# hangxu0304/DeepReduce

Measured on NVIDIA H100. Metric: ResNet-50 images/sec (whole job, device-timed, max over ranks), higher is better.
Workload: dtype bf16

## Files before the change

deepreduce_b200/models/fused_bn.py:

```python
from __future__ import annotations

import os

import torch
import torch.nn as nn
import torch.nn.functional as F


def enabled() -> bool:
    return os.environ.get("DR_FUSED_BN", "1") != "0"


def _eligible_x(x: torch.Tensor) -> bool:
    return (x.is_cuda and x.dtype == torch.bfloat16 and x.dim() == 4 and x.stride(1) == 1
            and x.is_contiguous(memory_format=torch.channels_last) and x.size(1) % 8 == 0 and x.size(1) <= 8192
            and x.numel() < 2 ** 31 - 1 and x.numel() // x.size(1) > 1)


def _eligible_bn(bn: nn.BatchNorm2d) -> bool:
    return (bn.training and bn.track_running_stats and bn.running_mean is not None and bn.momentum is not None
            and bn.affine)


def eligible(x: torch.Tensor, bn: nn.BatchNorm2d) -> bool:
# ... 25 lines not shown
        dx, dw, db = ops.cuda_module().bn_backward(0, _grad(gy), mask, x, [mean, invstd, weight])
        return dx, dw, db, None, None


class _BNAddReLU(torch.autograd.Function):

    @staticmethod
    def forward(ctx, x, weight, bias, mean, invstd, z, wz, bz, mz, iz):
        from .. import ops
        mod = ops.cuda_module()
        if wz is None:
            o, mask = mod.bn_apply(1, x, [mean, invstd, weight, bias], z)
            ctx.save_for_backward(x, weight, mean, invstd, mask)
        else:
            o, mask = mod.bn_apply(2, x, [mean, invstd, weight, bias], z, [mz, iz, wz, bz])
            ctx.save_for_backward(x, weight, mean, invstd, mask, z, wz, mz, iz)
        ctx.has_bn_z = wz is not None
        return o

    @staticmethod
    def backward(ctx, go):
        from .. import ops
        mod = ops.cuda_module()
        saved = ctx.saved_tensors
        x, weight, mean, invstd, mask = saved[:5]
        if not ctx.has_bn_z:
            dx, dw, db, g = mod.bn_backward(1, _grad(go), mask, x, [mean, invstd, weight])
            return dx, dw, db, None, None, g, None, None, None, None
        z, wz, mz, iz = saved[5:]
        dx, dw, db, dz, dwz, dbz = mod.bn_backward(2, _grad(go), mask, x, [mean, invstd, weight], z, [mz, iz, wz])
        return dx, dw, db, None, None, dz, dwz, dbz, None, None


def bn_relu(x: torch.Tensor, bn: nn.BatchNorm2d) -> torch.Tensor:
    if not eligible(x, bn):
        return F.relu(bn(x), inplace=True)
    mean, invstd = _stats(x, bn)
    return _BNReLU.apply(x, bn.weight, bn.bias, mean, invstd)


def bn_add_relu(x: torch.Tensor, bn: nn.BatchNorm2d, idt: torch.Tensor) -> torch.Tensor:
    if not (eligible(x, bn) and idt.dtype == x.dtype and idt.shape == x.shape and idt.stride() == x.stride()):
        return F.relu(bn(x) + idt, inplace=True)
    mean, invstd = _stats(x, bn)
    return _BNAddReLU.apply(x, bn.weight, bn.bias, mean, invstd, idt, None, None, None, None)


def bn_bn_add_relu(x: torch.Tensor, bn: nn.BatchNorm2d, xd: torch.Tensor, bnd: nn.BatchNorm2d) -> torch.Tensor:
    if not (eligible(x, bn) and eligible(xd, bnd) and xd.shape == x.shape and xd.stride() == x.stride()):
        return F.relu(bn(x) + bnd(xd), inplace=True)
    md, id_ = _stats(xd, bnd)
    mean, invstd = _stats(x, bn)
    return _BNAddReLU.apply(x, bn.weight, bn.bias, mean, invstd, xd, bnd.weight, bnd.bias, md, id_)
```

deepreduce_b200/models/resnet.py:

```python
from __future__ import annotations

import torch.nn as nn
import torch.nn.functional as F

from .fused_bn import bn_add_relu, bn_bn_add_relu, bn_relu


class _BasicCifar(nn.Module):
    def __init__(self, inp, out, stride):
        super().__init__()
        self.conv1 = nn.Conv2d(inp, out, 3, stride, 1, bias=False)
        self.bn1 = nn.BatchNorm2d(out)
        self.conv2 = nn.Conv2d(out, out, 3, 1, 1, bias=False)
        self.bn2 = nn.BatchNorm2d(out)
        self.pad = None
        if stride != 1 or inp != out:
            self.pad = (out - inp, stride)

    def forward(self, x):
        y = F.relu(self.bn1(self.conv1(x)))
        y = self.bn2(self.conv2(y))
        if self.pad is not None:
            extra, s = self.pad
            x = F.pad(x[:, :, ::s, ::s], (0, 0, 0, 0, extra // 2, extra - extra // 2))
        return F.relu(x + y)


class ResNetCifar(nn.Module):
    def __init__(self, n: int = 3, num_classes: int = 10):
        super().__init__()
        self.conv1 = nn.Conv2d(3, 16, 3, 1, 1, bias=False)
        self.bn1 = nn.BatchNorm2d(16)
        layers, inp = [], 16
        for out, stride in ((16, 1), (32, 2), (64, 2)):
            for i in range(n):
                layers.append(_BasicCifar(inp, out, stride if i == 0 else 1))
                inp = out
        self.layers = nn.Sequential(*layers)
# ... 25 lines not shown
        self.downsample = None
        if downsample:
            self.downsample = nn.Sequential(nn.Conv2d(inp, out, 1, stride, bias=False), nn.BatchNorm2d(out))

    def forward(self, x):
        xd = None if self.downsample is None else self.downsample[0](x)
        y = bn_relu(self.conv1(x), self.bn1)
        y = bn_relu(self.conv2(y), self.bn2)
        y = self.conv3(y)
        if xd is None:
            return bn_add_relu(y, self.bn3, x)
        return bn_bn_add_relu(y, self.bn3, xd, self.downsample[1])


class ResNet(nn.Module):
    def __init__(self, blocks=(3, 4, 6, 3), num_classes: int = 1000):
        super().__init__()
        self.conv1 = nn.Conv2d(3, 64, 7, 2, 3, bias=False)
        self.bn1 = nn.BatchNorm2d(64)
        self.maxpool = nn.MaxPool2d(3, 2, 1)
        stages, inp = [], 64
        for i, (n, width) in enumerate(zip(blocks, (64, 128, 256, 512))):
            for j in range(n):
                stride = 2 if (j == 0 and i > 0) else 1
                stages.append(_Bottleneck(inp, width, stride, downsample=(j == 0)))
                inp = width * 4
        self.layers = nn.Sequential(*stages)
        self.fc = nn.Linear(inp, num_classes)
        for m in self.modules():
            if isinstance(m, nn.Conv2d):
                nn.init.kaiming_normal_(m.weight, mode="fan_out", nonlinearity="relu")

    def forward(self, x):
        x = self.maxpool(bn_relu(self.conv1(x), self.bn1))
        x = self.layers(x)
        x = F.adaptive_avg_pool2d(x, 1).flatten(1)
        return self.fc(x)


def resnet50(num_classes: int = 1000) -> ResNet:
    return ResNet((3, 4, 6, 3), num_classes)
```

deepreduce_b200/ops/csrc/binding.cpp:

```cpp
#include <ATen/cuda/CUDAContext.h>
#include <c10/cuda/CUDAGuard.h>
#include <c10/cuda/CUDAStream.h>
#include <torch/extension.h>

#include <condition_variable>
#include <deque>
#include <mutex>
#include <thread>

#include "ops.h"

namespace py = pybind11;
using dr::EngineParams;

#define CHECK_CUDA_T(x) TORCH_CHECK((x).is_cuda() && (x).is_contiguous(), #x " must be a contiguous CUDA tensor")

static cudaStream_t cur_stream() { return at::cuda::getCurrentCUDAStream().stream(); }

static void check_last(const char* what) {
  cudaError_t e = cudaGetLastError();
  TORCH_CHECK(e == cudaSuccess, what, ": ", cudaGetErrorString(e));
}

static torch::Tensor bloom_insert(torch::Tensor idx, int64_t k, int64_t m_bits, int64_t seed) {
// ... 260 lines not shown
  for (int i = 0; i < 4; ++i) check_chan(p[i], C, names[i]);
  return {p[0].data_ptr<float>(), p[1].data_ptr<float>(), p[2].data_ptr<float>(), p[3].data_ptr<float>()};
}

static void check_like_x(const torch::Tensor& t, const torch::Tensor& x, const char* what) {
  TORCH_CHECK(t.sizes() == x.sizes() && t.strides() == x.strides() && t.scalar_type() == torch::kBFloat16 &&
                  t.device() == x.device(),
              "bn: ", what, " must match x in shape, layout, dtype and device");
}

static std::vector<torch::Tensor> bn_apply(int64_t mode, torch::Tensor x, std::vector<torch::Tensor> p,
                                           c10::optional<torch::Tensor> z, std::vector<torch::Tensor> pz) {
  check_bn_input(x);
  const int64_t C = x.size(1);
  const dr::BnParams px = bn_params(p, C);
  dr::BnParams pzz{};
  const void* zp = nullptr;
  if (mode != 0) {
    TORCH_CHECK(z.has_value(), "bn: mode ", mode, " needs z");
    check_like_x(*z, x, "z");
    zp = z->data_ptr();
    if (mode == 2) pzz = bn_params(pz, C);
  }
  c10::cuda::CUDAGuard g(x.device());
  const int64_t rows = x.numel() / C;
  auto out = torch::empty_like(x);
  auto mask = torch::empty({rows, C / 8}, x.options().dtype(torch::kUInt8));
  cudaError_t e = dr::launch_bn_apply((int)mode, x.data_ptr(), px, zp, pzz, out.data_ptr(), mask.data_ptr(), rows,
                                      (int)C, cur_stream());
  TORCH_CHECK(e == cudaSuccess, "bn_apply: ", cudaGetErrorString(e));
  return {out, mask};
}

static dr::BnParams bn_bwd_params(const std::vector<torch::Tensor>& p, int64_t C) {
  TORCH_CHECK(p.size() == 3, "bn_backward: expected (mean, invstd, weight)");
  const char* names[3] = {"mean", "invstd", "weight"};
  for (int i = 0; i < 3; ++i) check_chan(p[i], C, names[i]);
  return {p[0].data_ptr<float>(), p[1].data_ptr<float>(), p[2].data_ptr<float>(), nullptr};
}

static std::vector<torch::Tensor> bn_backward(int64_t mode, torch::Tensor go, torch::Tensor mask, torch::Tensor x,
                                              std::vector<torch::Tensor> p, c10::optional<torch::Tensor> z,
                                              std::vector<torch::Tensor> pz) {
  TORCH_CHECK(mode >= 0 && mode <= 2, "bn_backward: mode must be 0, 1 or 2");
  check_bn_input(x);
  TORCH_CHECK(go.sizes() == x.sizes() && go.scalar_type() == torch::kBFloat16 && go.device() == x.device() &&
                  go.is_contiguous(at::MemoryFormat::ChannelsLast),
              "bn_backward: go must be a channels_last bf16 tensor of x's shape on x's device");
  const int64_t C = x.size(1), rows = x.numel() / C;
  TORCH_CHECK(mask.is_cuda() && mask.scalar_type() == torch::kUInt8 && mask.is_contiguous() &&
                  mask.numel() == rows * (C / 8) && mask.device() == x.device(),
              "bn_backward: mask must be bn_apply's mask for x");
  c10::cuda::CUDAGuard guard(x.device());
  int block_y = 0, grid_y = 0;
  dr::bn_row_tree(rows, (int)C, &block_y, &grid_y);
  TORCH_CHECK((int64_t)block_y * grid_y <= rows, "bn_backward: reduction tree wider than the rows");
  const int n_sums = mode == 2 ? 3 : 2;
  auto f32 = x.options().dtype(torch::kFloat32);
  auto sums = torch::empty({n_sums, C}, f32);
  auto staging = grid_y > 1 ? torch::empty({n_sums, grid_y, C}, f32) : torch::Tensor();
  auto dx = torch::empty_like(x), dw = torch::empty({C}, f32), db = torch::empty({C}, f32);
  dr::BnBwd b{};
  b.go = go.data_ptr(); b.mask = mask.data_ptr<uint8_t>(); b.x = x.data_ptr();
  b.px = bn_bwd_params(p, C);
  b.dx = dx.data_ptr(); b.sums = sums.data_ptr<float>(); b.staging = grid_y > 1 ? staging.data_ptr<float>() : nullptr;
  b.dw = dw.data_ptr<float>(); b.db = db.data_ptr<float>();
  std::vector<torch::Tensor> res{dx, dw, db};
  if (mode == 1) {
    auto g = torch::empty_like(x);
    b.g = g.data_ptr();
    res.push_back(g);
  } else if (mode == 2) {
    TORCH_CHECK(z.has_value(), "bn_backward: mode 2 needs z");
    check_like_x(*z, x, "z");
    b.z = z->data_ptr();
    b.pz = bn_bwd_params(pz, C);
    auto dz = torch::empty_like(x), dwz = torch::empty({C}, f32), dbz = torch::empty({C}, f32);
    b.dz = dz.data_ptr(); b.dwz = dwz.data_ptr<float>(); b.dbz = dbz.data_ptr<float>();
    res.insert(res.end(), {dz, dwz, dbz});
  }
  cudaError_t e = dr::launch_bn_backward((int)mode, b, rows, (int)C, cur_stream());
  TORCH_CHECK(e == cudaSuccess, "bn_backward: ", cudaGetErrorString(e));
  return res;
}

struct Engine {
  EngineParams P{};
  int grid = 0;
  int grid_cap = 0;
  int blocks_per_sm = 2;
  int dyn_smem = 64 * 1024;
  int device = 0;

  Engine(int64_t tensors, int64_t tiles, int64_t n_tensors, int64_t n_tiles, int64_t slot_words,
         int64_t payload_words, int64_t grad, int64_t resid, int64_t hist, int64_t hist_total, int64_t sel,
         int64_t tile_count, int64_t barrier, int64_t status, std::vector<int64_t> arenas, int rank, int world) {
    TORCH_CHECK(world <= dr::kMaxWorld && (int)arenas.size() == world, "bad world/arenas");
    P.tensors = reinterpret_cast<const dr::TensorDesc*>(tensors);
    P.tiles = reinterpret_cast<const dr::TileInfo*>(tiles);
    P.n_tensors = (uint32_t)n_tensors; P.n_tiles = (uint32_t)n_tiles;
    P.slot_words = (uint32_t)slot_words; P.payload_words = (uint32_t)payload_words;
    P.grad = reinterpret_cast<float*>(grad); P.resid = reinterpret_cast<float*>(resid);
    P.hist = reinterpret_cast<uint32_t*>(hist); P.hist_total = reinterpret_cast<uint32_t*>(hist_total);
    P.sel = reinterpret_cast<dr::SelState*>(sel);
// ... 168 lines not shown
}
static int64_t arena_import(const std::string& b) {
  TORCH_CHECK(b.size() == sizeof(dr::ArenaHandle), "bad handle");
  dr::ArenaHandle h;
  memcpy(h.bytes, b.data(), sizeof(h.bytes));
  void* p = dr::arena_import(h);
  TORCH_CHECK(p != nullptr, "cudaIpcOpenMemHandle failed (peer access / IPC unavailable)");
  return (int64_t)p;
}
static torch::Tensor arena_as_tensor(int64_t p, int64_t n_words, int64_t device) {
  auto opts = torch::TensorOptions().dtype(torch::kInt32).device(torch::kCUDA, (int)device);
  return torch::from_blob((void*)p, {n_words}, opts);
}

PYBIND11_MODULE(TORCH_EXTENSION_NAME, m) {
  m.def("launch_count", [] { return (int64_t)dr::launch_count(); });
  m.def("bloom_insert", &bloom_insert);
  m.def("bloom_select", &bloom_select);
  m.def("qsgd_encode", &qsgd_encode);
  m.def("qsgd_decode", &qsgd_decode);
  m.def("pack_bits", &pack_bits);
  m.def("unpack_bits", &unpack_bits);
  m.def("polyfit_fit", &polyfit_fit);
  m.def("polyfit_eval", &polyfit_eval);
  m.def("dexp_fit", &dexp_fit);
  m.def("conflict_sets_pick", &conflict_sets_pick);
  m.def("delta_bp128_encode", &delta_bp128_encode);
  m.def("delta_bp128_decode", &delta_bp128_decode);
  m.def("u8_to_nhwc_norm", &u8_to_nhwc_norm);
  m.def("bn_stats", &bn_stats, py::arg("x"), py::arg("running_mean"), py::arg("running_var"), py::arg("momentum"),
        py::arg("eps"), py::arg("torch_kernel") = false);
  m.def("bn_apply", &bn_apply, py::arg("mode"), py::arg("x"), py::arg("p"), py::arg("z") = py::none(),
        py::arg("pz") = std::vector<torch::Tensor>{});
  m.def("bn_backward", &bn_backward, py::arg("mode"), py::arg("go"), py::arg("mask"), py::arg("x"), py::arg("p"),
        py::arg("z") = py::none(), py::arg("pz") = std::vector<torch::Tensor>{});
  m.def("rle_runs", &rle_runs);
  m.def("rle_indices", &rle_indices);
  m.def("arena_alloc", &arena_alloc);
  m.def("arena_free", [](int64_t p) { dr::arena_free((void*)p); });
  m.def("arena_export", &arena_export);
  m.def("arena_import", &arena_import);
  m.def("arena_close", [](int64_t p) { dr::arena_close((void*)p); });
  m.def("arena_as_tensor", &arena_as_tensor);
  m.def("enable_peer_access", [](std::vector<int> devices) { return dr::arena_enable_peer_access(devices.data(), (int)devices.size()); });
  m.attr("TILE") = dr::kTile;
  m.attr("ARENA_HDR_WORDS") = dr::kArenaHdrWords;
  m.attr("SLOT_HEADER_WORDS") = dr::kSlotHeaderWords;
  m.attr("HIST_BINS") = dr::kHistBins;
  m.attr("NUM_HIST") = dr::kNumHist;
  m.attr("PH_END") = (int)dr::kPhEnd;

  py::class_<Engine>(m, "Engine")
      .def(py::init<int64_t, int64_t, int64_t, int64_t, int64_t, int64_t, int64_t, int64_t, int64_t, int64_t, int64_t,
                    int64_t, int64_t, int64_t, std::vector<int64_t>, int, int>())
      .def("configure", &Engine::configure)
      .def("set_buffers", &Engine::set_buffers)
      .def("set_poly", &Engine::set_poly)
      .def("set_shard", &Engine::set_shard)
      .def("set_has_rle", &Engine::set_has_rle)
      .def("set_scratch", &Engine::set_scratch)
      .def("set_peer_timeout_ms", &Engine::set_peer_timeout_ms)
      .def("set_fault", &Engine::set_fault)
      .def("set_deterministic", &Engine::set_deterministic)
      .def("set_cost_prefix", &Engine::set_cost_prefix)
      .def("set_debug_times", &Engine::set_debug_times)
      .def("set_cuts", &Engine::set_cuts)
// ... 12 lines not shown
```

deepreduce_b200/ops/csrc/bn.cu:

```cuda
#include <cuda_bf16.h>

#include <algorithm>

#include "common.cuh"
#include "ops.h"

namespace dr {

namespace {

constexpr int kVec = 8;
constexpr int kApplyThreads = 256;
constexpr int kReduceThreads = 128;

struct ChanParams {
  float m[kVec], inv[kVec], w[kVec], b[kVec];
};

__device__ __forceinline__ void load8(const float* __restrict__ p, float* d) {
  const float4 a = __ldg(reinterpret_cast<const float4*>(p));
  const float4 b = __ldg(reinterpret_cast<const float4*>(p) + 1);
  d[0] = a.x; d[1] = a.y; d[2] = a.z; d[3] = a.w;
  d[4] = b.x; d[5] = b.y; d[6] = b.z; d[7] = b.w;
}
// ... 25 lines not shown
  const int c = (threadIdx.x % groups) * kVec;
  ChanParams a;
  load_params(px, c, a);
  ChanParams d;
  if (kMode == 2) load_params(pz, c, d);
  const int64_t step = (int64_t)gridDim.x * rows_per_cta;
#pragma unroll 2
  for (int64_t r = (int64_t)blockIdx.x * rows_per_cta + rsub; r < rows; r += step) {
    const int64_t off = r * C + c;
    const uint4 vx = *reinterpret_cast<const uint4*>(x + off);
    uint4 vz = make_uint4(0, 0, 0, 0);
    if (kMode != 0) vz = *reinterpret_cast<const uint4*>(z + off);
    const __nv_bfloat16* hx = reinterpret_cast<const __nv_bfloat16*>(&vx);
    const __nv_bfloat16* hz = reinterpret_cast<const __nv_bfloat16*>(&vz);
    uint4 vo;
    __nv_bfloat16* ho = reinterpret_cast<__nv_bfloat16*>(&vo);
    unsigned bits = 0;
#pragma unroll
    for (int i = 0; i < kVec; ++i) {
      __nv_bfloat16 y = __float2bfloat16_rn(bn_elem(__bfloat162float(hx[i]), a.m[i], a.inv[i], a.w[i], a.b[i]));
      if (kMode != 0) {
        const __nv_bfloat16 s = kMode == 1 ? hz[i]
                                           : __float2bfloat16_rn(bn_elem(__bfloat162float(hz[i]), d.m[i], d.inv[i], d.w[i], d.b[i]));
        y = __float2bfloat16_rn(__fadd_rn(__bfloat162float(y), __bfloat162float(s)));
      }
      ho[i] = relu_bf16(y);
      bits |= (__bfloat162float(ho[i]) <= 0.f ? 0u : 1u) << i;
    }
    *reinterpret_cast<uint4*>(out + off) = vo;
    mask[r * groups + c / kVec] = (uint8_t)bits;
  }
}

struct RowTree {
  int block_y, grid_y;
  __host__ __device__ int S() const { return block_y * grid_y; }
  __host__ __device__ int loops(int rows) const { return 1 + (rows - 1) / (S() * kLoads); }
  static constexpr int kLoads = 4;
};

constexpr int kStatsThreads = 256;

__device__ __forceinline__ void welford_update(float x, float inv, float valid, float& mean, float& m2n) {
  const float d0 = __fsub_rn(x, mean);
  mean = __fmaf_rn(d0, inv, mean);
  const float d1 = __fsub_rn(x, mean);
  m2n = __fmaf_rn(__fmul_rn(d0, d1), valid, m2n);
}

template <int kN, bool kFuseNew>
__device__ __forceinline__ void welford_merge(int& n, float* mean, float* m2n, int n_new, const float* mean_new,
                                              const float* m2n_new) {
  const float fn = (float)n, fn_new = (float)n_new;
  const float factor = __frcp_rn((float)max(1, n + n_new));
#pragma unroll
  for (int i = 0; i < kN; ++i) {
    const float d = __fsub_rn(mean[i], mean_new[i]);
    const float s = kFuseNew ? __fmaf_rn(mean_new[i], fn_new, __fmul_rn(mean[i], fn))
                             : __fmaf_rn(mean[i], fn, __fmul_rn(mean_new[i], fn_new));
    mean[i] = __fmul_rn(s, factor);
    const float u = __fmul_rn(__fmul_rn(__fmul_rn(d, d), fn_new), fn);
    m2n[i] = __fadd_rn(m2n[i], __fmaf_rn(u, factor, m2n_new[i]));
  }
  n += n_new;
}

// ... 183 lines not shown
  const int group = blockIdx.x * gpc + tg;
  const bool live = group * kVec < C;
  const int c = live ? group * kVec : 0;
  const int S = t.S();
  float m[kVec], mz[kVec];
#pragma unroll
  for (int i = 0; i < kVec; ++i) {
    m[i] = mean[c + i];
    mz[i] = kMode == 2 ? mean_z[c + i] : 0.f;
  }
  float acc[kSums][L][kVec];
#pragma unroll
  for (int k = 0; k < kSums; ++k)
#pragma unroll
    for (int j = 0; j < L; ++j)
#pragma unroll
      for (int i = 0; i < kVec; ++i) acc[k][j][i] = 0.f;
  const int mgroups = C / kVec;
  int r = blockIdx.y * t.block_y + y;
  const int n_loops = t.loops(rows);
  struct Batch {
    uint4 g[L], x[L], z[L];
    unsigned m[L];
  };
  auto load = [&](Batch& b, int r0) {
#pragma unroll
    for (int j = 0; j < L; ++j) {
      const int rr = r0 + j * S;
      if (live && rr < rows) {
        const int off = rr * C + c;
        b.g[j] = *reinterpret_cast<const uint4*>(go + off);
        b.x[j] = *reinterpret_cast<const uint4*>(x + off);
        if (kMode == 2) b.z[j] = *reinterpret_cast<const uint4*>(z + off);
        b.m[j] = mask[rr * mgroups + group];
      } else {
        b.g[j] = uint4{}; b.x[j] = uint4{}; b.z[j] = uint4{}; b.m[j] = 0;
      }
    }
  };
  Batch cur;
  load(cur, r);
  for (int it = 0; it < n_loops; ++it) {
    Batch nxt;
    load(nxt, r + L * S);
    const unsigned* mb = cur.m;
#pragma unroll
    for (int j = 0; j < L; ++j) {
      const __nv_bfloat16* hg = reinterpret_cast<const __nv_bfloat16*>(&cur.g[j]);
      const __nv_bfloat16* hx = reinterpret_cast<const __nv_bfloat16*>(&cur.x[j]);
      const __nv_bfloat16* hz = reinterpret_cast<const __nv_bfloat16*>(&cur.z[j]);
      uint4 vo;
      __nv_bfloat16* ho = reinterpret_cast<__nv_bfloat16*>(&vo);
#pragma unroll
      for (int i = 0; i < kVec; ++i) {
        const unsigned bit = (mb[j] >> i) & 1u;
        const float g = masked(hg[i], bit);
        if (kMode == 1) ho[i] = bit ? hg[i] : __float2bfloat16_rn(0.f);
        acc[0][j][i] = __fadd_rn(acc[0][j][i], g);
        acc[1][j][i] = __fmaf_rn(__fsub_rn(__bfloat162float(hx[i]), m[i]), g, acc[1][j][i]);
        if (kMode == 2) acc[2][j][i] = __fmaf_rn(__fsub_rn(__bfloat162float(hz[i]), mz[i]), g, acc[2][j][i]);
      }
      if (kMode == 1 && live && r + j * S < rows) *reinterpret_cast<uint4*>(g_out + (r + j * S) * C + c) = vo;
    }
    cur = nxt;
    r += L * S;
  }
#pragma unroll
  for (int k = 0; k < kSums; ++k) {
#pragma unroll
    for (int i = 0; i < kVec; ++i)
#pragma unroll
      for (int j = 1; j < L; ++j) acc[k][0][i] = __fadd_rn(acc[k][0][i], acc[k][j][i]);
    tree_over_y<kVec>(acc[k][0], sh, y, t.block_y, tg * kVec, gpc * kVec);
  }
  if (y != 0 || !live) return;
#pragma unroll
  for (int k = 0; k < kSums; ++k)
#pragma unroll
    for (int i = 0; i < kVec; ++i) {
      if (t.grid_y > 1) o.staging[((size_t)k * t.grid_y + blockIdx.y) * C + c + i] = acc[k][0][i];
      else bwd_store(o, k, c + i, C, acc[k][0][i], invstd, invstd_z);
    }
}

__global__ void bn_bwd_finalize_kernel(BwdOut o, RowTree t, int n_sums, int C, const float* __restrict__ invstd,
                                       const float* __restrict__ invstd_z) {
  extern __shared__ float sh[];
  const int cols = blockDim.x / t.block_y;
  const int col = threadIdx.x % cols, y = threadIdx.x / cols;
// ... 28 lines not shown

__device__ __forceinline__ __nv_bfloat16 elemt(float g, float x, const ElemtChan& p, int i, float norm) {
  const float a = __fmaf_rn(-p.sdy[i], norm, g);
  return __float2bfloat16_rn(__fmul_rn(__fmaf_rn(-p.f1[i], __fsub_rn(x, p.m[i]), a), p.f2[i]));
}

struct ElemtArgs {
  const float *mean, *invstd, *weight, *sums;
  const float *mean_z, *invstd_z, *weight_z;
};

template <int kMode>
__global__ void __launch_bounds__(kApplyThreads) bn_bwd_elemt_kernel(const __nv_bfloat16* __restrict__ g_in,
                                                                     const uint8_t* __restrict__ mask,
                                                                     const __nv_bfloat16* __restrict__ x,
                                                                     const __nv_bfloat16* __restrict__ z, ElemtArgs a,
                                                                     __nv_bfloat16* __restrict__ dx,
                                                                     __nv_bfloat16* __restrict__ dz, float norm,
                                                                     int64_t rows, int C) {
  const int groups = C / kVec;
  const int rows_per_cta = blockDim.x / groups;
  const int rsub = threadIdx.x / groups;
  if (rsub >= rows_per_cta) return;
  const int c = (threadIdx.x % groups) * kVec;
  ElemtChan p;
  elemt_params(a.mean, a.invstd, a.weight, a.sums, a.sums + C, norm, c, p);
  ElemtChan q;
  if (kMode == 2) elemt_params(a.mean_z, a.invstd_z, a.weight_z, a.sums, a.sums + 2 * C, norm, c, q);
  const int64_t step = (int64_t)gridDim.x * rows_per_cta;
#pragma unroll 2
  for (int64_t r = (int64_t)blockIdx.x * rows_per_cta + rsub; r < rows; r += step) {
    const int64_t off = r * C + c;
    const uint4 vg = *reinterpret_cast<const uint4*>(g_in + off);
    const uint4 vx = *reinterpret_cast<const uint4*>(x + off);
    uint4 vz = make_uint4(0, 0, 0, 0);
    if (kMode == 2) vz = *reinterpret_cast<const uint4*>(z + off);
    const unsigned mb = kMode == 1 ? 0xffu : mask[r * groups + c / kVec];
    const __nv_bfloat16* hg = reinterpret_cast<const __nv_bfloat16*>(&vg);
    const __nv_bfloat16* hx = reinterpret_cast<const __nv_bfloat16*>(&vx);
    const __nv_bfloat16* hz = reinterpret_cast<const __nv_bfloat16*>(&vz);
    uint4 vo, vd;
    __nv_bfloat16* ho = reinterpret_cast<__nv_bfloat16*>(&vo);
    __nv_bfloat16* hd = reinterpret_cast<__nv_bfloat16*>(&vd);
#pragma unroll
    for (int i = 0; i < kVec; ++i) {
      const float g = masked(hg[i], (mb >> i) & 1u);
      ho[i] = elemt(g, __bfloat162float(hx[i]), p, i, norm);
      if (kMode == 2) hd[i] = elemt(g, __bfloat162float(hz[i]), q, i, norm);
    }
    *reinterpret_cast<uint4*>(dx + off) = vo;
    if (kMode == 2) *reinterpret_cast<uint4*>(dz + off) = vd;
  }
}

__global__ void bn_update_stats_kernel(const float* __restrict__ mean, float* __restrict__ var_invstd,
                                       float* __restrict__ running_mean, float* __restrict__ running_var, int C,
                                       float momentum, float bessel, float eps) {
  const int c = blockIdx.x * blockDim.x + threadIdx.x;
  if (c >= C) return;
  const float m = mean[c], v = var_invstd[c];
  const float unbiased_var = v * bessel;
  running_mean[c] = m * momentum + (1 - momentum) * running_mean[c];
  running_var[c] = unbiased_var * momentum + (1 - momentum) * running_var[c];
  var_invstd[c] = rsqrtf(v + eps);
}

template <typename K>
cudaError_t rows_grid(K kernel, int64_t rows, int C, int& grid, int& threads) {
  const int groups = C / kVec;
  const int rows_per_cta = groups >= kApplyThreads ? 1 : kApplyThreads / groups;
// ... 27 lines not shown
  return std::max<int>(1, (int)(n - (n >> 1)));
}

RowTree row_tree(int rows, int C) {
  const int block_x = std::min(last_pow2((unsigned)C), 32);
  const int block_y = std::min(last_pow2((unsigned)((rows + 15) / 16)), 512 / block_x);
  int grid_y = std::min((rows + block_y * 16 - 1) / (block_y * 16), 128);
  if (grid_y < 8) grid_y = 1;
  return {block_y, grid_y};
}

template <int kMode>
cudaError_t launch_bwd_reduce(const BnBwd& b, const RowTree& t, const BwdOut& o, int rows, int C, cudaStream_t st) {
  const int groups = C / kVec;
  const int gpc = std::min(groups, std::max(1, kReduceThreads / t.block_y));
  const dim3 grid((groups + gpc - 1) / gpc, t.grid_y);
  const int threads = gpc * t.block_y;
  count_launch();
  bn_bwd_reduce_kernel<kMode><<<grid, threads, threads * kVec * sizeof(float), st>>>(
      reinterpret_cast<const __nv_bfloat16*>(b.go), b.mask, reinterpret_cast<const __nv_bfloat16*>(b.x), b.px.mean,
      b.px.invstd, reinterpret_cast<const __nv_bfloat16*>(b.z), b.pz.mean, b.pz.invstd,
      reinterpret_cast<__nv_bfloat16*>(b.g), o, t, rows, C);
  return cudaGetLastError();
}

template <int kMode>
cudaError_t launch_bwd_elemt(const BnBwd& b, const ElemtArgs& a, int64_t rows, int C, cudaStream_t st) {
  int grid = 0, threads = 0;
  cudaError_t e = rows_grid(bn_bwd_elemt_kernel<kMode>, rows, C, grid, threads);
  if (e != cudaSuccess) return e;
  const float norm = (float)(1.0 / (double)rows);
  count_launch();
  bn_bwd_elemt_kernel<kMode><<<grid, threads, 0, st>>>(
      reinterpret_cast<const __nv_bfloat16*>(kMode == 1 ? b.g : b.go), b.mask,
      reinterpret_cast<const __nv_bfloat16*>(b.x), reinterpret_cast<const __nv_bfloat16*>(b.z), a,
      reinterpret_cast<__nv_bfloat16*>(b.dx), reinterpret_cast<__nv_bfloat16*>(b.dz), norm, rows, C);
  return cudaGetLastError();
}

template <int kMode>
cudaError_t launch_backward(const BnBwd& b, int64_t rows64, int C, cudaStream_t st) {
  const int rows = (int)rows64;
  const RowTree t = row_tree(rows, C);
  const BwdOut o{b.sums, b.dw, b.db, b.dwz, b.dbz, b.staging};
  cudaError_t e = launch_bwd_reduce<kMode>(b, t, o, rows, C, st);
  if (e != cudaSuccess) return e;
  if (t.grid_y > 1) {
    const int cols = std::max(1, 512 / t.block_y);
    const int threads = cols * t.block_y;
    count_launch();
    bn_bwd_finalize_kernel<<<(C + cols - 1) / cols, threads, threads * sizeof(float), st>>>(
        o, t, kMode == 2 ? 3 : 2, C, b.px.invstd, b.pz.invstd);
    e = cudaGetLastError();
    if (e != cudaSuccess) return e;
  }
  const ElemtArgs a{b.px.mean, b.px.invstd, b.px.weight, b.sums, b.pz.mean, b.pz.invstd, b.pz.weight};
  return launch_bwd_elemt<kMode>(b, a, rows64, C, st);
}

cudaError_t launch_stats(const BnStats& s, int rows, int C, cudaStream_t st) {
  const RowTree t = row_tree(rows, C);
  const int grid_y = t.grid_y;
  const StatsOut o{s.mean, s.invstd, s.running_mean, s.running_var,
                   s.staging, s.staging + (size_t)grid_y * C, reinterpret_cast<int*>(s.staging + 2 * (size_t)grid_y * C),
                   s.momentum, s.bessel, s.eps};
  const int groups = C / kVec;
  const int gpc = std::min(groups, std::max(1, kStatsThreads / (RowTree::kLoads * t.block_y)));
  const int threads = gpc * RowTree::kLoads * t.block_y;
  count_launch();
  bn_stats_kernel<<<dim3((groups + gpc - 1) / gpc, grid_y), threads, WelfordSlots<kVec>::bytes(threads), st>>>(
      reinterpret_cast<const __nv_bfloat16*>(s.x), o, t, rows, C);
  cudaError_t e = cudaGetLastError();
  if (e != cudaSuccess || grid_y == 1) return e;
  const int cols = std::max(1, 512 / t.block_y);
  const int fthreads = cols * t.block_y;
  count_launch();
  bn_stats_finalize_kernel<<<(C + cols - 1) / cols, fthreads, WelfordSlots<1>::bytes(fthreads), st>>>(o, t, C);
  return cudaGetLastError();
}

}

void bn_row_tree(int64_t rows, int C, int* block_y, int* grid_y) {
  const RowTree t = row_tree((int)rows, C);
  *block_y = t.block_y;
  *grid_y = t.grid_y;
}

cudaError_t launch_bn_backward(int mode, const BnBwd& b, int64_t rows, int C, cudaStream_t st) {
  if (rows == 0) return cudaSuccess;
  switch (mode) {
    case 0: return launch_backward<0>(b, rows, C, st);
    case 1: return launch_backward<1>(b, rows, C, st);
    case 2: return launch_backward<2>(b, rows, C, st);
    default: return cudaErrorInvalidValue;
  }
}

cudaError_t launch_bn_stats(const BnStats& s, int64_t rows, int C, cudaStream_t st) {
  if (rows == 0) return cudaSuccess;
  return launch_stats(s, (int)rows, C, st);
}

cudaError_t launch_bn_update_stats(const float* mean, float* var_invstd, float* running_mean, float* running_var, int C,
                                   float momentum, float bessel, float eps, cudaStream_t st) {
  count_launch();
  bn_update_stats_kernel<<<(C + 255) / 256, 256, 0, st>>>(mean, var_invstd, running_mean, running_var, C, momentum,
                                                          bessel, eps);
  return cudaGetLastError();
}

cudaError_t launch_bn_apply(int mode, const void* x, const BnParams& px, const void* z, const BnParams& pz, void* out,
                            void* mask, int64_t rows, int C, cudaStream_t st) {
  switch (mode) {
    case 0: return launch_apply<0>(x, px, z, pz, out, mask, rows, C, st);
    case 1: return launch_apply<1>(x, px, z, pz, out, mask, rows, C, st);
    case 2: return launch_apply<2>(x, px, z, pz, out, mask, rows, C, st);
    default: return cudaErrorInvalidValue;
  }
}

}
```

deepreduce_b200/ops/csrc/ops.h:

```cpp
#pragma once
#include <cuda_runtime.h>
#include <stdint.h>

#include "plan.h"

namespace dr {

int engine_max_grid(int blocks_per_sm, int dyn_smem_bytes);
cudaError_t engine_launch(const EngineParams& P, int grid, int blocks_per_sm, int dyn_smem_bytes, cudaStream_t stream);
void count_launch(int n);
long long launch_count();

void launch_bloom_insert(const int64_t* idx, int64_t n, uint32_t* filter, uint32_t n_hash, uint32_t m_bits,
                         uint32_t seed, cudaStream_t st);
void launch_bloom_count(const uint32_t* filter, uint32_t d, uint32_t n_hash, uint32_t m_bits, uint32_t seed,
                        uint32_t* tile_counts, uint32_t* tile_excl, cudaStream_t st);
void launch_bloom_emit(const uint32_t* filter, uint32_t d, uint32_t n_hash, uint32_t m_bits, uint32_t seed,
                       const uint32_t* tile_excl, int64_t* out, uint32_t limit, cudaStream_t st);
void launch_qsgd_encode(const float* v, int64_t K, int bucket, int q, uint32_t seed, void* lvl, bool i16, float* norms,
                        cudaStream_t st);
void launch_qsgd_decode(const void* lvl, bool i16, const float* norms, int64_t K, int bucket, int q, float* out,
                        cudaStream_t st);
void launch_pack_bits(const int64_t* vals, int64_t n, int bits, uint32_t* out, int64_t n_words, cudaStream_t st);
void launch_unpack_bits(const uint32_t* in, int64_t n_words, int64_t n, int bits, int64_t* out, cudaStream_t st);
// ... 7 lines not shown
void launch_bp128_widths(const int64_t* idx, int64_t n, uint32_t* widths, cudaStream_t st);
void launch_bp128_pack(const int64_t* idx, int64_t n, const uint32_t* widths, const int64_t* word_off, uint32_t* out,
                       cudaStream_t st);
void launch_bp128_unpack(const uint32_t* in, int64_t n, int64_t* word_off, int64_t* deltas, cudaStream_t st);
void launch_rle_count(const int64_t* idx, int64_t n, uint32_t* counts, uint32_t* excl, cudaStream_t st);
void launch_rle_runs(const int64_t* idx, int64_t n, const uint32_t* excl, int64_t* start_pos, int64_t* end_pos,
                     int64_t n_runs, int64_t d, int64_t* runs, cudaStream_t st);
void launch_rle_expand(const int64_t* ones_excl, const int64_t* run_start, int64_t n_runs, int64_t total, int64_t* out,
                       cudaStream_t st);

struct ArenaHandle { unsigned char bytes[64]; };
void* arena_alloc(size_t bytes);
void arena_free(void* p);
ArenaHandle arena_export(void* p);
void* arena_import(const ArenaHandle& h);
void arena_close(void* p);
int arena_enable_peer_access(const int* devices, int n);
void launch_u8_to_nhwc_norm(const uint8_t* in, void* out_bf16, int64_t n_pix, const float* mean, const float* inv_std,
                            cudaStream_t st);

struct BnParams { const float* mean; const float* invstd; const float* weight; const float* bias; };
void bn_row_tree(int64_t rows, int C, int* block_y, int* grid_y);
struct BnStats {
  const void* x;
  float* mean; float* invstd; float* running_mean; float* running_var;
  float* staging;
  float momentum, bessel, eps;
};
cudaError_t launch_bn_stats(const BnStats& s, int64_t rows, int C, cudaStream_t st);
cudaError_t launch_bn_update_stats(const float* mean, float* var_invstd, float* running_mean, float* running_var, int C,
                                   float momentum, float bessel, float eps, cudaStream_t st);
cudaError_t launch_bn_apply(int mode, const void* x, const BnParams& px, const void* z, const BnParams& pz, void* out,
                            void* mask, int64_t rows, int C, cudaStream_t st);
struct BnBwd {
  const void* go; const uint8_t* mask; const void* x; const void* z;
  BnParams px, pz;
  void* dx; void* dz; void* g;
  float* sums; float* staging; float* dw; float* db; float* dwz; float* dbz;
};
cudaError_t launch_bn_backward(int mode, const BnBwd& b, int64_t rows, int C, cudaStream_t st);

}
```

Measured before the change: 4850.

## Fuse stem BatchNorm, ReLU and 3x3 max-pool into one kernel with backward

Adds a fused kernel that applies the stem BatchNorm and ReLU and then the 3x3 stride-2 max-pool in a single pass. It writes the pooled output plus per-element argmax/sign codes instead of the full-resolution activation and ReLU mask. Backward gets a new mode that scatters pooled gradients through the codes into a full-resolution buffer before the existing BN backward reduce and elementwise kernels. This removes the full-size stem activation write and read and the separate max-pool kernels, at the cost of each input being reloaded by up to four overlapping pooling windows and more complex backward indexing.

```diff
diff --git a/deepreduce_b200/models/fused_bn.py b/deepreduce_b200/models/fused_bn.py
--- a/deepreduce_b200/models/fused_bn.py
+++ b/deepreduce_b200/models/fused_bn.py
@@ -81,6 +81,38 @@
         return dx, dw, db, None, None, dz, dwz, dbz, None, None
 
 
+class _BNReLUMaxPool(torch.autograd.Function):
+
+    @staticmethod
+    def forward(ctx, x, weight, bias, mean, invstd):
+        from .. import ops
+        out, codes = ops.cuda_module().bn_apply_pool(x, [mean, invstd, weight, bias])
+        ctx.save_for_backward(x, weight, mean, invstd, codes)
+        return out
+
+    @staticmethod
+    def backward(ctx, go):
+        from .. import ops
+        x, weight, mean, invstd, codes = ctx.saved_tensors
+        dx, dw, db = ops.cuda_module().bn_backward(3, _grad(go), codes, x, [mean, invstd, weight])
+        return dx, dw, db, None, None
+
+
+def _stem_pool(pool: nn.Module) -> bool:
+    if type(pool) is not nn.MaxPool2d:
+        return False
+    pair = lambda v: tuple(v) if isinstance(v, (tuple, list)) else (v, v)
+    return (pair(pool.kernel_size) == (3, 3) and pair(pool.stride) == (2, 2) and pair(pool.padding) == (1, 1)
+            and pair(pool.dilation) == (1, 1) and not pool.ceil_mode and not pool.return_indices)
+
+
+def bn_relu_maxpool(x: torch.Tensor, bn: nn.BatchNorm2d, pool: nn.MaxPool2d) -> torch.Tensor:
+    if not (eligible(x, bn) and _stem_pool(pool)):
+        return pool(F.relu(bn(x), inplace=True))
+    mean, invstd = _stats(x, bn)
+    return _BNReLUMaxPool.apply(x, bn.weight, bn.bias, mean, invstd)
+
+
 def bn_relu(x: torch.Tensor, bn: nn.BatchNorm2d) -> torch.Tensor:
     if not eligible(x, bn):
         return F.relu(bn(x), inplace=True)
diff --git a/deepreduce_b200/models/resnet.py b/deepreduce_b200/models/resnet.py
--- a/deepreduce_b200/models/resnet.py
+++ b/deepreduce_b200/models/resnet.py
@@ -3,7 +3,7 @@
 import torch.nn as nn
 import torch.nn.functional as F
 
-from .fused_bn import bn_add_relu, bn_bn_add_relu, bn_relu
+from .fused_bn import bn_add_relu, bn_bn_add_relu, bn_relu, bn_relu_maxpool
 
 
 class _BasicCifar(nn.Module):
@@ -95,7 +95,7 @@
                 nn.init.kaiming_normal_(m.weight, mode="fan_out", nonlinearity="relu")
 
     def forward(self, x):
-        x = self.maxpool(bn_relu(self.conv1(x), self.bn1))
+        x = bn_relu_maxpool(self.conv1(x), self.bn1, self.maxpool)
         x = self.layers(x)
         x = F.adaptive_avg_pool2d(x, 1).flatten(1)
         return self.fc(x)
diff --git a/deepreduce_b200/ops/csrc/binding.cpp b/deepreduce_b200/ops/csrc/binding.cpp
--- a/deepreduce_b200/ops/csrc/binding.cpp
+++ b/deepreduce_b200/ops/csrc/binding.cpp
@@ -316,6 +316,23 @@
   return {out, mask};
 }
 
+static std::vector<torch::Tensor> bn_apply_pool(torch::Tensor x, std::vector<torch::Tensor> p, int64_t kernel_size,
+                                                int64_t stride, int64_t padding, int64_t dilation, bool ceil_mode) {
+  TORCH_CHECK(kernel_size == 3 && stride == 2 && padding == 1 && dilation == 1 && !ceil_mode,
+              "bn_apply_pool: only kernel 3, stride 2, padding 1, dilation 1, floor mode");
+  check_bn_input(x);
+  const int64_t N = x.size(0), C = x.size(1), H = x.size(2), W = x.size(3);
+  const dr::BnParams px = bn_params(p, C);
+  c10::cuda::CUDAGuard g(x.device());
+  const dr::PoolGeom pg{(int)H, (int)W, (int)((H - 1) / 2 + 1), (int)((W - 1) / 2 + 1)};
+  auto out = torch::empty({N, C, pg.Ho, pg.Wo}, x.options().memory_format(at::MemoryFormat::ChannelsLast));
+  auto codes = torch::empty({N * pg.Ho * pg.Wo, C}, x.options().dtype(torch::kUInt8));
+  cudaError_t e = dr::launch_bn_apply_pool(x.data_ptr(), px, out.data_ptr(), codes.data_ptr(), (int)N, pg, (int)C,
+                                           cur_stream());
+  TORCH_CHECK(e == cudaSuccess, "bn_apply_pool: ", cudaGetErrorString(e));
+  return {out, codes};
+}
+
 static dr::BnParams bn_bwd_params(const std::vector<torch::Tensor>& p, int64_t C) {
   TORCH_CHECK(p.size() == 3, "bn_backward: expected (mean, invstd, weight)");
   const char* names[3] = {"mean", "invstd", "weight"};
@@ -326,15 +343,20 @@
 static std::vector<torch::Tensor> bn_backward(int64_t mode, torch::Tensor go, torch::Tensor mask, torch::Tensor x,
                                               std::vector<torch::Tensor> p, c10::optional<torch::Tensor> z,
                                               std::vector<torch::Tensor> pz) {
-  TORCH_CHECK(mode >= 0 && mode <= 2, "bn_backward: mode must be 0, 1 or 2");
+  TORCH_CHECK(mode >= 0 && mode <= 3, "bn_backward: mode must be 0, 1, 2 or 3");
   check_bn_input(x);
-  TORCH_CHECK(go.sizes() == x.sizes() && go.scalar_type() == torch::kBFloat16 && go.device() == x.device() &&
+  const int64_t C = x.size(1), rows = x.numel() / C;
+  dr::PoolGeom pg{(int)x.size(2), (int)x.size(3), (int)((x.size(2) - 1) / 2 + 1), (int)((x.size(3) - 1) / 2 + 1)};
+  const std::vector<int64_t> go_shape =
+      mode == 3 ? std::vector<int64_t>{x.size(0), C, pg.Ho, pg.Wo} : x.sizes().vec();
+  TORCH_CHECK(go.sizes() == go_shape && go.scalar_type() == torch::kBFloat16 && go.device() == x.device() &&
                   go.is_contiguous(at::MemoryFormat::ChannelsLast),
-              "bn_backward: go must be a channels_last bf16 tensor of x's shape on x's device");
-  const int64_t C = x.size(1), rows = x.numel() / C;
+              "bn_backward: go must be a channels_last bf16 tensor on x's device, of x's shape (mode 3: the pooled "
+              "shape)");
+  const int64_t mask_numel = mode == 3 ? go.numel() : rows * (C / 8);
   TORCH_CHECK(mask.is_cuda() && mask.scalar_type() == torch::kUInt8 && mask.is_contiguous() &&
-                  mask.numel() == rows * (C / 8) && mask.device() == x.device(),
-              "bn_backward: mask must be bn_apply's mask for x");
+                  mask.numel() == mask_numel && mask.device() == x.device(),
+              "bn_backward: mask must be bn_apply's mask (mode 3: bn_apply_pool's codes) for x");
   c10::cuda::CUDAGuard guard(x.device());
   int block_y = 0, grid_y = 0;
   dr::bn_row_tree(rows, (int)C, &block_y, &grid_y);
@@ -349,11 +371,13 @@
   b.px = bn_bwd_params(p, C);
   b.dx = dx.data_ptr(); b.sums = sums.data_ptr<float>(); b.staging = grid_y > 1 ? staging.data_ptr<float>() : nullptr;
   b.dw = dw.data_ptr<float>(); b.db = db.data_ptr<float>();
+  b.pool = pg;
   std::vector<torch::Tensor> res{dx, dw, db};
-  if (mode == 1) {
-    auto g = torch::empty_like(x);
+  torch::Tensor g;
+  if (mode == 1 || mode == 3) {
+    g = torch::empty_like(x);
     b.g = g.data_ptr();
-    res.push_back(g);
+    if (mode == 1) res.push_back(g);
   } else if (mode == 2) {
     TORCH_CHECK(z.has_value(), "bn_backward: mode 2 needs z");
     check_like_x(*z, x, "z");
@@ -588,6 +612,8 @@
         py::arg("eps"), py::arg("torch_kernel") = false);
   m.def("bn_apply", &bn_apply, py::arg("mode"), py::arg("x"), py::arg("p"), py::arg("z") = py::none(),
         py::arg("pz") = std::vector<torch::Tensor>{});
+  m.def("bn_apply_pool", &bn_apply_pool, py::arg("x"), py::arg("p"), py::arg("kernel_size") = 3, py::arg("stride") = 2,
+        py::arg("padding") = 1, py::arg("dilation") = 1, py::arg("ceil_mode") = false);
   m.def("bn_backward", &bn_backward, py::arg("mode"), py::arg("go"), py::arg("mask"), py::arg("x"), py::arg("p"),
         py::arg("z") = py::none(), py::arg("pz") = std::vector<torch::Tensor>{});
   m.def("rle_runs", &rle_runs);
diff --git a/deepreduce_b200/ops/csrc/bn.cu b/deepreduce_b200/ops/csrc/bn.cu
--- a/deepreduce_b200/ops/csrc/bn.cu
+++ b/deepreduce_b200/ops/csrc/bn.cu
@@ -81,6 +81,153 @@
   }
 }
 
+
+__global__ void __launch_bounds__(kApplyThreads) bn_apply_pool_kernel(const __nv_bfloat16* __restrict__ x, BnParams px,
+                                                                      __nv_bfloat16* __restrict__ out,
+                                                                      uint8_t* __restrict__ codes, int64_t orows,
+                                                                      PoolGeom pg, int C) {
+  const int groups = C / kVec;
+  const int rows_per_cta = blockDim.x / groups;
+  const int rsub = threadIdx.x / groups;
+  if (rsub >= rows_per_cta) return;
+  const int c = (threadIdx.x % groups) * kVec;
+  ChanParams a;
+  load_params(px, c, a);
+  const int64_t step = (int64_t)gridDim.x * rows_per_cta;
+  for (int64_t r = (int64_t)blockIdx.x * rows_per_cta + rsub; r < orows; r += step) {
+    const int ow = (int)(r % pg.Wo);
+    const int64_t t = r / pg.Wo;
+    const int oh = (int)(t % pg.Ho);
+    const int64_t n = t / pg.Ho;
+    const int h0 = 2 * oh - 1, w0 = 2 * ow - 1;
+    uint4 v[9];
+#pragma unroll
+    for (int k = 0; k < 9; ++k) {
+      const int ih = h0 + k / 3, iw = w0 + k % 3;
+      v[k] = ih >= 0 && ih < pg.H && iw >= 0 && iw < pg.W
+                 ? *reinterpret_cast<const uint4*>(x + ((n * pg.H + ih) * pg.W + iw) * C + c)
+                 : uint4{};
+    }
+    __nv_bfloat16 best[kVec];
+    unsigned slot[kVec];
+#pragma unroll
+    for (int i = 0; i < kVec; ++i) {
+      best[i] = __float2bfloat16_rn(-INFINITY);
+      slot[i] = 0;
+    }
+#pragma unroll
+    for (int k = 0; k < 9; ++k) {
+      const int ih = h0 + k / 3, iw = w0 + k % 3;
+      if (ih < 0 || ih >= pg.H || iw < 0 || iw >= pg.W) continue;
+      const __nv_bfloat16* hx = reinterpret_cast<const __nv_bfloat16*>(&v[k]);
+#pragma unroll
+      for (int i = 0; i < kVec; ++i) {
+        const __nv_bfloat16 y = relu_bf16(__float2bfloat16_rn(bn_elem(__bfloat162float(hx[i]), a.m[i], a.inv[i], a.w[i], a.b[i])));
+        const float fy = __bfloat162float(y);
+        if (fy > __bfloat162float(best[i]) || isnan(fy)) {
+          best[i] = y;
+          slot[i] = k;
+        }
+      }
+    }
+    uint4 vo;
+    __nv_bfloat16* ho = reinterpret_cast<__nv_bfloat16*>(&vo);
+    uint2 vc;
+    uint8_t* hc = reinterpret_cast<uint8_t*>(&vc);
+#pragma unroll
+    for (int i = 0; i < kVec; ++i) {
+      ho[i] = best[i];
+      hc[i] = (uint8_t)(slot[i] | (__bfloat162float(best[i]) <= 0.f ? 0u : 0x80u));
+    }
+    *reinterpret_cast<uint4*>(out + r * C + c) = vo;
+    *reinterpret_cast<uint2*>(codes + r * C + c) = vc;
+  }
+}
+
+struct PoolGather {
+  uint4 g[4];
+  uint2 code[4];
+  int off;
+  int nh, nw;
+  int sh, sw;
+};
+
+__device__ __forceinline__ void pool_gather_codes(PoolGather& q, const uint8_t* __restrict__ codes, const PoolGeom& pg,
+                                                  int row, int C, int c, bool valid) {
+  const int w = row % pg.W, t = row / pg.W, h = t % pg.H, n = t / pg.H;
+  const int ph = h >> 1, pw = w >> 1;
+  q.nh = valid ? min((h + 1) / 2 + 1, pg.Ho) - ph : 0;
+  q.nw = valid ? min((w + 1) / 2 + 1, pg.Wo) - pw : 0;
+  q.sh = h - 2 * ph + 1;
+  q.sw = w - 2 * pw + 1;
+  q.off = ((n * pg.Ho + ph) * pg.Wo + pw) * C + c;
+#pragma unroll
+  for (int k = 0; k < 4; ++k) {
+    const int a = k >> 1, b = k & 1;
+    q.code[k] = a < q.nh && b < q.nw ? *reinterpret_cast<const uint2*>(codes + q.off + (a * pg.Wo + b) * C) : uint2{};
+  }
+}
+
+__device__ __forceinline__ void pool_gather_grads(PoolGather& q, const __nv_bfloat16* __restrict__ gp,
+                                                  const PoolGeom& pg, int C) {
+#pragma unroll
+  for (int k = 0; k < 4; ++k) {
+    const int a = k >> 1, b = k & 1;
+    q.g[k] = a < q.nh && b < q.nw ? *reinterpret_cast<const uint4*>(gp + q.off + (a * pg.Wo + b) * C) : uint4{};
+  }
+}
+
+__device__ __forceinline__ void pool_gather_resolve(const PoolGather& q, uint4& g, unsigned& bits) {
+  __nv_bfloat16* hg = reinterpret_cast<__nv_bfloat16*>(&g);
+  const bool single = q.nh == 1 && q.nw == 1;
+  bits = 0;
+#pragma unroll
+  for (int i = 0; i < kVec; ++i) {
+    float s = 0.f;
+    __nv_bfloat16 one = __float2bfloat16_rn(0.f);
+    unsigned bit = 0;
+#pragma unroll
+    for (int k = 0; k < 4; ++k) {
+      const int a = k >> 1, b = k & 1;
+      const unsigned code = (reinterpret_cast<const uint8_t*>(&q.code[k]))[i];
+      if (a < q.nh && b < q.nw && (int)(code & 0x7fu) == (q.sh - 2 * a) * 3 + (q.sw - 2 * b)) {
+        const __nv_bfloat16 v = (reinterpret_cast<const __nv_bfloat16*>(&q.g[k]))[i];
+        s = __fadd_rn(s, __bfloat162float(v));
+        one = v;
+        bit = code >> 7;
+      }
+    }
+    hg[i] = single ? one : __float2bfloat16_rn(s);
+    bits |= bit << i;
+  }
+}
+
+__global__ void __launch_bounds__(kApplyThreads) bn_pool_grad_kernel(const __nv_bfloat16* __restrict__ gp,
+                                                                     const uint8_t* __restrict__ codes,
+                                                                     __nv_bfloat16* __restrict__ g, PoolGeom pg,
+                                                                     int64_t rows, int C) {
+  const int groups = C / kVec;
+  const int rows_per_cta = blockDim.x / groups;
+  const int rsub = threadIdx.x / groups;
+  if (rsub >= rows_per_cta) return;
+  const int c = (threadIdx.x % groups) * kVec;
+  const int64_t step = (int64_t)gridDim.x * rows_per_cta;
+#pragma unroll 2
+  for (int64_t r = (int64_t)blockIdx.x * rows_per_cta + rsub; r < rows; r += step) {
+    PoolGather q;
+    pool_gather_codes(q, codes, pg, (int)r, C, c, true);
+    pool_gather_grads(q, gp, pg, C);
+    uint4 v;
+    unsigned bits;
+    pool_gather_resolve(q, v, bits);
+    __nv_bfloat16* hv = reinterpret_cast<__nv_bfloat16*>(&v);
+#pragma unroll
+    for (int i = 0; i < kVec; ++i)
+      if (!((bits >> i) & 1u)) hv[i] = __float2bfloat16_rn(0.f);
+    *reinterpret_cast<uint4*>(g + r * C + c) = v;
+  }
+}
+
 struct RowTree {
   int block_y, grid_y;
   __host__ __device__ int S() const { return block_y * grid_y; }
@@ -330,7 +477,7 @@
         b.g[j] = *reinterpret_cast<const uint4*>(go + off);
         b.x[j] = *reinterpret_cast<const uint4*>(x + off);
         if (kMode == 2) b.z[j] = *reinterpret_cast<const uint4*>(z + off);
-        b.m[j] = mask[rr * mgroups + group];
+        b.m[j] = kMode == 3 ? 0u : mask[rr * mgroups + group];
       } else {
         b.g[j] = uint4{}; b.x[j] = uint4{}; b.z[j] = uint4{}; b.m[j] = 0;
       }
@@ -352,7 +499,7 @@
 #pragma unroll
       for (int i = 0; i < kVec; ++i) {
         const unsigned bit = (mb[j] >> i) & 1u;
-        const float g = masked(hg[i], bit);
+        const float g = kMode == 3 ? __bfloat162float(hg[i]) : masked(hg[i], bit);
         if (kMode == 1) ho[i] = bit ? hg[i] : __float2bfloat16_rn(0.f);
         acc[0][j][i] = __fadd_rn(acc[0][j][i], g);
         acc[1][j][i] = __fmaf_rn(__fsub_rn(__bfloat162float(hx[i]), m[i]), g, acc[1][j][i]);
@@ -447,10 +594,10 @@
   for (int64_t r = (int64_t)blockIdx.x * rows_per_cta + rsub; r < rows; r += step) {
     const int64_t off = r * C + c;
     const uint4 vg = *reinterpret_cast<const uint4*>(g_in + off);
+    const unsigned mb = kMode == 1 || kMode == 3 ? 0xffu : mask[r * groups + c / kVec];
     const uint4 vx = *reinterpret_cast<const uint4*>(x + off);
     uint4 vz = make_uint4(0, 0, 0, 0);
     if (kMode == 2) vz = *reinterpret_cast<const uint4*>(z + off);
-    const unsigned mb = kMode == 1 ? 0xffu : mask[r * groups + c / kVec];
     const __nv_bfloat16* hg = reinterpret_cast<const __nv_bfloat16*>(&vg);
     const __nv_bfloat16* hx = reinterpret_cast<const __nv_bfloat16*>(&vx);
     const __nv_bfloat16* hz = reinterpret_cast<const __nv_bfloat16*>(&vz);
@@ -544,7 +691,7 @@
   const float norm = (float)(1.0 / (double)rows);
   count_launch();
   bn_bwd_elemt_kernel<kMode><<<grid, threads, 0, st>>>(
-      reinterpret_cast<const __nv_bfloat16*>(kMode == 1 ? b.g : b.go), b.mask,
+      reinterpret_cast<const __nv_bfloat16*>(kMode == 1 || kMode == 3 ? b.g : b.go), b.mask,
       reinterpret_cast<const __nv_bfloat16*>(b.x), reinterpret_cast<const __nv_bfloat16*>(b.z), a,
       reinterpret_cast<__nv_bfloat16*>(b.dx), reinterpret_cast<__nv_bfloat16*>(b.dz), norm, rows, C);
   return cudaGetLastError();
@@ -555,7 +702,20 @@
   const int rows = (int)rows64;
   const RowTree t = row_tree(rows, C);
   const BwdOut o{b.sums, b.dw, b.db, b.dwz, b.dbz, b.staging};
-  cudaError_t e = launch_bwd_reduce<kMode>(b, t, o, rows, C, st);
+  cudaError_t e;
+  if (kMode == 3) {
+    int grid = 0, threads = 0;
+    e = rows_grid(bn_pool_grad_kernel, rows64, C, grid, threads);
+    if (e != cudaSuccess) return e;
+    count_launch();
+    bn_pool_grad_kernel<<<grid, threads, 0, st>>>(reinterpret_cast<const __nv_bfloat16*>(b.go), b.mask,
+                                                  reinterpret_cast<__nv_bfloat16*>(b.g), b.pool, rows64, C);
+    e = cudaGetLastError();
+    if (e != cudaSuccess) return e;
+  }
+  BnBwd bb = b;
+  if (kMode == 3) bb.go = b.g;
+  e = launch_bwd_reduce<kMode>(bb, t, o, rows, C, st);
   if (e != cudaSuccess) return e;
   if (t.grid_y > 1) {
     const int cols = std::max(1, 512 / t.block_y);
@@ -605,6 +765,7 @@
     case 0: return launch_backward<0>(b, rows, C, st);
     case 1: return launch_backward<1>(b, rows, C, st);
     case 2: return launch_backward<2>(b, rows, C, st);
+    case 3: return launch_backward<3>(b, rows, C, st);
     default: return cudaErrorInvalidValue;
   }
 }
@@ -632,4 +793,18 @@
   }
 }
 
-}
+cudaError_t launch_bn_apply_pool(const void* x, const BnParams& px, void* out, void* codes, int N, const PoolGeom& pg,
+                                 int C, cudaStream_t st) {
+  const int64_t orows = (int64_t)N * pg.Ho * pg.Wo;
+  if (orows == 0) return cudaSuccess;
+  int grid = 0, threads = 0;
+  cudaError_t e = rows_grid(bn_apply_pool_kernel, orows, C, grid, threads);
+  if (e != cudaSuccess) return e;
+  count_launch();
+  bn_apply_pool_kernel<<<grid, threads, 0, st>>>(reinterpret_cast<const __nv_bfloat16*>(x), px,
+                                                 reinterpret_cast<__nv_bfloat16*>(out),
+                                                 reinterpret_cast<uint8_t*>(codes), orows, pg, C);
+  return cudaGetLastError();
+}
+
+}
diff --git a/deepreduce_b200/ops/csrc/ops.h b/deepreduce_b200/ops/csrc/ops.h
--- a/deepreduce_b200/ops/csrc/ops.h
+++ b/deepreduce_b200/ops/csrc/ops.h
@@ -63,11 +63,15 @@
                                    float momentum, float bessel, float eps, cudaStream_t st);
 cudaError_t launch_bn_apply(int mode, const void* x, const BnParams& px, const void* z, const BnParams& pz, void* out,
                             void* mask, int64_t rows, int C, cudaStream_t st);
+struct PoolGeom { int H, W, Ho, Wo; };
+cudaError_t launch_bn_apply_pool(const void* x, const BnParams& px, void* out, void* codes, int N, const PoolGeom& pg,
+                                 int C, cudaStream_t st);
 struct BnBwd {
   const void* go; const uint8_t* mask; const void* x; const void* z;
   BnParams px, pz;
   void* dx; void* dz; void* g;
   float* sums; float* staging; float* dw; float* db; float* dwz; float* dbz;
+  PoolGeom pool;
 };
 cudaError_t launch_bn_backward(int mode, const BnBwd& b, int64_t rows, int C, cudaStream_t st);
 
```

Measured after the change: 5066, median of 6. 1.04x the previous value.
